# evoldoers/machineboss

Measured on NVIDIA B200. Metric: forward_viterbi_gcups, higher is better.
Workload: dtype f64

## Files before the change

machineboss_b200/csrc/mb_api.cu:

```cuda
#include <algorithm>
#include <cmath>
#include <cstdio>
#include <cstring>
#include <mutex>

#include "mb_internal.h"

namespace mb {

static thread_local std::string g_error;
static thread_local int g_device = 0;
static thread_local int g_forceEngine = -1;
static thread_local Options g_options;

static const char* const kOptionNames[] = {
  "verbose",
  "jit_narrow", "jit_no_linear", "jit_c", "jit_cv", "jit_minblocks", "jit_minblocks_v", "jit_minblocks_linv", "jit_minblocks_lin", "jit_minblocks_cnt", "jit_threads",
  "jit_tb_budget_mb", "jit_f_budget_mb",
  "jit_chunks",
  "jit_no_norm",
  "jit_unroll",
  "jit_fit_c",
  "jit_split",
  "lane_r", "lane_warps", "no_lane", "lane_old", "lane_bs", "lane_la", "lane_wn", "lane_host_only", "lane_warps_per_cta", "wide_g", "wide_w", "no_big", "big_warps", "big_debug", "big_no_fold", "big_early_store", "big_smem_kb",
  "no_col", "col_no_traceback", "col_bp_budget_mb", "col_c", "col_sil_regs", "col_threads", "col_minblocks", "col_r", "col_bnd_budget_mb",
};

Options thread_options() { return g_options; }
void set_thread_options (const Options& o) { g_options = o; }
int thread_engine() { return g_forceEngine; }

bool option_known (const char* name) {
  for (const char* n: kOptionNames) if (!strcmp (n, name)) return true;
  return false;
}

void set_error (const std::string& msg) { g_error = msg; }

bool cuda_ok (cudaError_t e, const char* what) {
  if (e == cudaSuccess) return true;
  set_error (std::string ("CUDA error: ") + cudaGetErrorString (e) + " in " + what);
  return false;
}

int timing_begin (mb_batch* b) {
  b->lastMs = 0;
  b->lastLaunches = 0;
  MB_CUDA (cudaEventRecord (b->evStart, b->stream));
  return 0;
}

int timing_end (mb_batch* b, int64_t launches) {
  MB_CUDA (cudaEventRecord (b->evStop, b->stream));
// ... 797 lines not shown
```

machineboss_b200/csrc/mb_jit.cu:

```cuda
#include <cuda.h>
#include <dlfcn.h>
#include <nvrtc.h>
#include <unistd.h>

#include <algorithm>
#include <cmath>
#include <cstdio>
#include <cstring>
#include <map>
#include <mutex>
#include <sstream>

#include "mb_internal.h"
#include "mb_jit_skeleton.h"

namespace mb {

struct Driver {
  CUresult (*ModuleLoadData) (CUmodule*, const void*) = nullptr;
  CUresult (*ModuleUnload) (CUmodule) = nullptr;
  CUresult (*ModuleGetFunction) (CUfunction*, CUmodule, const char*) = nullptr;
  CUresult (*ModuleGetGlobal) (CUdeviceptr*, size_t*, CUmodule, const char*) = nullptr;
  CUresult (*LaunchKernel) (CUfunction, unsigned, unsigned, unsigned, unsigned, unsigned, unsigned, unsigned, CUstream, void**, void**) = nullptr;
  CUresult (*FuncSetAttribute) (CUfunction, CUfunction_attribute, int) = nullptr;
// ... 62 lines not shown
      || !g_nvrtc.GetProgramLog || !g_nvrtc.DestroyProgram) { set_error ("libnvrtc is missing symbols"); return false; }
  g_nvrtc.ok = true;
  return true;
}

static bool cu_ok (CUresult r, const char* what) {
  if (r == CUDA_SUCCESS) return true;
  const char* s = nullptr;
  if (g_drv.GetErrorString) g_drv.GetErrorString (r, &s);
  set_error (std::string ("CUDA driver error: ") + (s ? s : "?") + " in " + what);
  return false;
}

struct Slot {
  int type, self, other, rank;
  int emitOff = -1;
  int silIdx = -1;
  int idOff = 0;
  int tableSize = 1;
};

struct Program {
  std::vector<Slot> slots;
  std::vector<int> stateSlot0;
  std::vector<int32_t> idTab;
  std::vector<int32_t> emitId;
  std::vector<int32_t> silId;
  int nEmit = 0, nSil = 0;
  int WA = 0, WB = 0;
  std::vector<int> rowOff;
  std::vector<int32_t> rowId;
  std::vector<int> rowSlot;
  std::vector<int> unitSlot;
};

static int table_size (int type, int nIn, int nOut) {
  return type == T_MATCH ? nIn * nOut : type == T_DELETE ? nIn : type == T_INSERT ? nOut : 1;
}

static int label_index (int type, int a, int b, int nOut) {
  return type == T_MATCH ? (a - 1) * nOut + (b - 1) : type == T_DELETE ? a - 1 : type == T_INSERT ? b - 1 : 0;
}

static int trans_type (int a, int b) { return a ? (b ? T_MATCH : T_DELETE) : (b ? T_INSERT : T_SILENT); }

static void build_program (const mb_machine* m, bool forward, Program& p) {
  struct Key { int self, type, other, rank; bool operator< (const Key& k) const { return std::tie (self, type, other, rank) < std::tie (k.self, k.type, k.other, k.rank); } };
  std::map<Key, std::vector<std::pair<int, int>>> groups;
  std::map<std::tuple<int, int, int, int>, int> seen;
  for (int64_t t = 0; t < m->T; ++t) {
    const int type = trans_type (m->in[t], m->out[t]);
    if (type == T_SILENT && m->dst[t] <= m->src[t]) continue;
    const int self = forward ? m->dst[t] : m->src[t], other = forward ? m->src[t] : m->dst[t];
    const int li = label_index (type, m->in[t], m->out[t], m->nOut);
    const int rank = seen[std::make_tuple (self, type, other, li)]++;
    groups[Key { self, type, other, rank }].push_back ({ li, (int) t });
  }
  p.stateSlot0.assign ((size_t) m->S + 1, 0);
  for (auto& g: groups) {
    Slot s;
    s.type = g.first.type; s.self = g.first.self; s.other = g.first.other; s.rank = g.first.rank;
    s.tableSize = table_size (s.type, m->nIn, m->nOut);
    s.idOff = (int) p.idTab.size();
    p.idTab.resize (p.idTab.size() + s.tableSize, -1);
    for (auto& e: g.second) p.idTab[s.idOff + e.first] = e.second;
    if (s.type == T_SILENT) { s.silIdx = p.nSil++; p.silId.push_back (g.second[0].second); }
    else {
      s.emitOff = p.nEmit;
      p.nEmit += s.tableSize;
      p.emitId.resize ((size_t) p.nEmit, -1);
      for (auto& e: g.second) p.emitId[s.emitOff + e.first] = e.second;
    }
    p.stateSlot0[s.self + 1]++;
    p.slots.push_back (s);
  }
  for (int s = 0; s < m->S; ++s) p.stateSlot0[s + 1] += p.stateSlot0[s];
  p.rowOff.assign (p.slots.size(), -1);
  for (size_t k = 0; k < p.slots.size(); ++k) {
    const Slot& sl = p.slots[k];
    if (sl.type == T_MATCH) { p.rowOff[k] = p.WA; p.WA += m->nOut; }
    else if (sl.type == T_DELETE) { p.rowOff[k] = p.WA; p.WA += 1; }
    else if (sl.type == T_INSERT) { p.rowOff[k] = p.WB; p.WB += 1; }
  }
  p.rowId.assign ((size_t) std::max (m->nIn * p.WA + m->nOut * p.WB, 1), -1);
  p.rowSlot.assign (p.rowId.size(), -1);
  for (size_t k = 0; k < p.slots.size(); ++k) {
    const Slot& sl = p.slots[k];
    auto put = [&] (int entry, int label) { p.rowId[entry] = p.idTab[sl.idOff + label]; p.rowSlot[entry] = (int) k; };
    if (sl.type == T_MATCH) { for (int a = 0; a < m->nIn; ++a) for (int b = 0; b < m->nOut; ++b) put (a * p.WA + p.rowOff[k] + b, a * m->nOut + b); }
    else if (sl.type == T_DELETE) { for (int a = 0; a < m->nIn; ++a) put (a * p.WA + p.rowOff[k], a); }
    else if (sl.type == T_INSERT) { for (int b = 0; b < m->nOut; ++b) put (m->nIn * p.WA + b * p.WB + p.rowOff[k], b); }
  }
  p.unitSlot.assign ((size_t) m->S, -1);
  for (int d = 0; d < m->S; ++d)
    for (int k = p.stateSlot0[d]; k < p.stateSlot0[d + 1]; ++k)
      if (p.slots[k].type == T_SILENT) { p.unitSlot[d] = k; break; }
}

struct JitEngine {
  Program fwd, bwd;
  int C = 4, tbBytes = 1, threads = 128, minBlocks = 4, minBlocksLin = 5, minBlocksCnt = 4;
  int CV = 4, minBlocksV = 4;
  int minBlocksLinV = 4;
  CUfunction kViterbiN = nullptr, kForwardLinN = nullptr, kBackwardLinN = nullptr, kViterbiScoreN = nullptr;
  int blocksPerSMN[4] = { 1, 1, 1, 1 };
  CUfunction kViterbiScore = nullptr;
  double* dRowVit = nullptr;
  double* dRowFLinN = nullptr;
  double* dRowBLinN = nullptr;
  std::vector<char> silParamLinN;
  bool normOK = false;
  std::string sourceV;
  struct FitModule { int C = 0; CUmodule mod = nullptr; CUfunction k[4] = { nullptr, nullptr, nullptr, nullptr }; int blocksPerSM[4] = { 1, 1, 1, 1 }; };
  std::vector<FitModule> fit;
  std::vector<int> fitFailed;
  std::string sourceS;
  CUmodule modS = nullptr;
  bool splitTried = false;
  CUfunction kSplit[4] = { nullptr, nullptr, nullptr, nullptr };
  int blocksPerSMS[4] = { 1, 1, 1, 1 };
  std::vector<int> stored;
  int storeQ = 1;
  CUmodule modV = nullptr;
  std::vector<int> shift, bits;
// ... 83 lines not shown
  for (auto& sl: p.slots) isSource[sl.other] = 1;
  for (int d = 0; d < m->S; ++d) {
    const int s0 = p.stateSlot0[d], s1 = p.stateSlot0[d + 1];
    const bool sinkOnly = !isSource[d] && d != 0 && s0 != s1;
    if (s0 == s1 || sinkOnly) o << "  double n" << d << " = mb_neg_inf();\n";
    if (sinkOnly) o << "  if (sink) {\n";
    for (int k = s0; k < s1; ++k) {
      const Slot& sl = p.slots[k];
      std::ostringstream t;
      t << source_expr (sl) << " + ";
      if (sl.type == T_SILENT) t << "P.f[" << sl.silIdx << "]"; else t << row_weight (sl, p.rowOff[k]);
      if (k == s0) o << (sinkOnly ? "  n" : "  double n") << d << " = " << t.str() << ";\n";
      else {
        const unsigned field = (unsigned) ((1ull << J.bits[d]) - 1ull), val = (unsigned) (k - s0);
        o << "  mb_vmax<PTR> (n" << d << ", " << t.str() << ", pk[(sh + " << J.shift[d] << ") >> 5], " << field << "u << ((sh + " << J.shift[d] << ") & 31), "
          << val << "u << ((sh + " << J.shift[d] << ") & 31));\n";
      }
    }
    if (sinkOnly) o << "  }\n";
    if (d == 0) o << "  if (origin) n" << d << " = 0.0;\n";
  }
  for (int d = 0; d < m->S; ++d) o << "  N[" << d << "] = n" << d << ";\n";
  o << "}\n\n";
}

static void gen_cell_row_lin (std::ostringstream& o, const mb_machine* m, const Program& p, bool forward) {
  o << "__device__ __forceinline__ void " << (forward ? "mb_cell_fwd_linr" : "mb_cell_bwd_linr")
    << " (const double (&D)[MB_S], const double (&L)[MB_S], const double (&U)[MB_S], double (&N)[MB_S], "
       "const unsigned ea, const unsigned em, const unsigned ebr, const bool origin, const MBSilN& P) {\n";
  const int originState = forward ? 0 : m->S - 1;
  for (int q = 0; q < m->S; ++q) {
    const int d = forward ? q : m->S - 1 - q;
    const int s0 = p.stateSlot0[d], s1 = p.stateSlot0[d + 1], unit = p.unitSlot[d];
    if (s0 == s1) o << "  double n" << d << " = 0.0;\n";
    if (unit >= 0) o << "  double n" << d << " = " << source_expr (p.slots[unit]) << ";\n";
    bool first = unit < 0;
    for (int k = s0; k < s1; ++k) {
      if (k == unit) continue;
      const Slot& sl = p.slots[k];
      std::ostringstream w;
      if (sl.type == T_SILENT) w << "P." << (forward ? "f" : "b") << "[" << sl.silIdx << "]"; else w << row_weight (sl, p.rowOff[k]);
      if (first) o << "  double n" << d << " = " << source_expr (sl) << " * " << w.str() << ";\n";
      else o << "  n" << d << " = fma (" << source_expr (sl) << ", " << w.str() << ", n" << d << ");\n";
      first = false;
    }
    if (d == originState) o << "  if (origin) n" << d << " = P." << (forward ? "originF" : "originB") << ";\n";
  }
  for (int d = 0; d < m->S; ++d) o << "  N[" << d << "] = n" << d << ";\n";
  o << "}\n\n";
}

static int ctx_count (int type, int C, int nOut) { return type == T_MATCH ? C * nOut : type == T_DELETE ? C : type == T_INSERT ? nOut : 0; }

static void gen_cell_counts (std::ostringstream& o, const mb_machine* m, const JitEngine& J) {
  const Program& p = J.bwd;
  o << "__device__ __forceinline__ void mb_cell_cnt (const double (&D)[MB_S], const double (&L)[MB_S], const double (&U)[MB_S], double (&N)[MB_S], const int a, const int b, const bool origin, const double* __restrict__ E, const MBSil& P, const double (&F)[MB_S], float (&cs)[MB_NSIL_B > 0 ? MB_NSIL_B : 1], float* __restrict__ acc, const int c) {\n";
  for (int q = 0; q < m->S; ++q) {
    const int d = m->S - 1 - q;
    const int s0 = p.stateSlot0[d], s1 = p.stateSlot0[d + 1];
    if (s0 == s1) o << "  double n" << d << " = mb_neg_inf();\n";
    for (int k = s0; k < s1; ++k) {
      const Slot& sl = p.slots[k];
      o << "  const double t" << k << " = " << term_expr (sl, m->nOut, false) << ";\n";
      if (k == s0) o << "  double n" << d << " = t" << k << ";\n";
      else o << "  n" << d << " = mb_lse (n" << d << ", t" << k << ");\n";
      o << "  { const float p = mb_post (F[" << d << "] + t" << k << "); ";
      if (sl.type == T_SILENT) o << "cs[" << sl.silIdx << "] += p; }\n";
      else {
        o << "acc[(" << J.ctxBase[k] << " + ";
        if (sl.type == T_MATCH) o << "c * " << m->nOut << " + b";
        else if (sl.type == T_DELETE) o << "c";
        else o << "b";
        o << ") * 32] += p; }\n";
      }
    }
    if (d == m->S - 1) o << "  if (origin) n" << d << " = 0.0;\n";
// ... 209 lines not shown
      fclose (f);
      if (!ok || rename (tmp.c_str(), cached.c_str())) remove (tmp.c_str());
    }
  }
  if (const char* d = getenv ("MB_JIT_DUMP")) { FILE* f = fopen ((std::string (d) + dumpSuffix + ".cubin").c_str(), "wb"); if (f) { fwrite (cubin.data(), 1, n, f); fclose (f); } }
  return 0;
}

static int compile (mb_machine* m, JitEngine& J) {
  std::vector<char> cubin, cubinV;
  if (nvrtc_compile (J.source, "", cubin, nullptr) || !load_driver()) return 1;
  if (!J.sourceV.empty() && nvrtc_compile (J.sourceV, ".viterbi.cu", cubinV, nullptr)) return 1;
  MB_CUDA (cudaFree (0));
  if (!cu_ok (g_drv.ModuleLoadData (&J.mod, cubin.data()), "cuModuleLoadData")) return 1;
  if (!J.sourceV.empty() && !cu_ok (g_drv.ModuleLoadData (&J.modV, cubinV.data()), "cuModuleLoadData")) return 1;
  if (!cu_ok (g_drv.ModuleGetFunction (&J.kForward, J.mod, "mb_k_forward"), "cuModuleGetFunction")
      || !cu_ok (g_drv.ModuleGetFunction (&J.kBackward, J.mod, "mb_k_backward"), "cuModuleGetFunction")
      || !cu_ok (g_drv.ModuleGetFunction (&J.kViterbi, J.modV ? J.modV : J.mod, "mb_k_viterbi"), "cuModuleGetFunction")
      || !cu_ok (g_drv.ModuleGetFunction (&J.kViterbiScore, J.modV ? J.modV : J.mod, "mb_k_viterbi_score"), "cuModuleGetFunction")
      || !cu_ok (g_drv.ModuleGetFunction (&J.kFStore, J.mod, "mb_k_fstore"), "cuModuleGetFunction")
      || !cu_ok (g_drv.ModuleGetFunction (&J.kBCounts, J.mod, "mb_k_bcounts"), "cuModuleGetFunction")
      || !cu_ok (g_drv.ModuleGetFunction (&J.kForwardLin, J.modV ? J.modV : J.mod, "mb_k_forward_lin"), "cuModuleGetFunction")
      || !cu_ok (g_drv.ModuleGetFunction (&J.kBackwardLin, J.modV ? J.modV : J.mod, "mb_k_backward_lin"), "cuModuleGetFunction")
      || !cu_ok (g_drv.ModuleGetFunction (&J.kFStoreLin, J.mod, "mb_k_fstore_lin"), "cuModuleGetFunction")
      || !cu_ok (g_drv.ModuleGetFunction (&J.kBCountsLin, J.mod, "mb_k_bcounts_lin"), "cuModuleGetFunction")) return 1;
  if (J.modV && (!cu_ok (g_drv.ModuleGetFunction (&J.kViterbiN, J.mod, "mb_k_viterbi"), "cuModuleGetFunction")
                 || !cu_ok (g_drv.ModuleGetFunction (&J.kViterbiScoreN, J.mod, "mb_k_viterbi_score"), "cuModuleGetFunction")
                 || !cu_ok (g_drv.ModuleGetFunction (&J.kForwardLinN, J.mod, "mb_k_forward_lin"), "cuModuleGetFunction")
                 || !cu_ok (g_drv.ModuleGetFunction (&J.kBackwardLinN, J.mod, "mb_k_backward_lin"), "cuModuleGetFunction"))) return 1;
  int dev = 0;
  MB_CUDA (cudaGetDevice (&dev));
  MB_CUDA (cudaDeviceGetAttribute (&J.numSMs, cudaDevAttrMultiProcessorCount, dev));
  CUfunction fn[10] = { J.kForward, J.kBackward, J.kViterbi, J.kFStore, J.kBCounts, J.kForwardLin, J.kBackwardLin, J.kFStoreLin, J.kBCountsLin, J.kViterbiScore };
  const int ne[10] = { J.fwd.nEmit, J.bwd.nEmit, J.fwd.nEmit, J.fwd.nEmit, J.bwd.nEmit, J.fwd.nEmit, J.bwd.nEmit, J.fwd.nEmit, J.bwd.nEmit, J.fwd.nEmit };
  for (int q = 0; q < 10; ++q) {
    const bool needAcc = q == 4 || q == 8;
    J.smemBytes[q] = (size_t) (((ne[q] + 1) & ~1) + (J.threads / 32) * (16 + 32 * (m->S + 1))) * 8
      + (needAcc ? (size_t) (J.threads / 32) * 32 * std::max (J.nCtx, 1) * (q == 8 ? 8 : 4) : 0)
      + (q == 8 ? (size_t) (J.threads / 32) * 2 * (32 * J.C * J.storeQ * 4) * 4 : 0);
    if (!cu_ok (g_drv.FuncSetAttribute (fn[q], CU_FUNC_ATTRIBUTE_MAX_DYNAMIC_SHARED_SIZE_BYTES, (int) J.smemBytes[q]), "cuFuncSetAttribute")) return 1;
    int nb = 0;
    if (!cu_ok (g_drv.OccupancyMaxActiveBlocksPerMultiprocessor (&nb, fn[q], J.threads, J.smemBytes[q]), "occupancy")) return 1;
    J.blocksPerSM[q] = std::max (1, nb);
  }
  if (J.modV) {
    CUfunction fnN[4] = { J.kViterbiN, J.kForwardLinN, J.kBackwardLinN, J.kViterbiScoreN };
    const int qOf[4] = { 2, 5, 6, 9 };
    for (int q = 0; q < 4; ++q) {
      if (!cu_ok (g_drv.FuncSetAttribute (fnN[q], CU_FUNC_ATTRIBUTE_MAX_DYNAMIC_SHARED_SIZE_BYTES, (int) J.smemBytes[qOf[q]]), "cuFuncSetAttribute")) return 1;
      int nb = 0;
      if (!cu_ok (g_drv.OccupancyMaxActiveBlocksPerMultiprocessor (&nb, fnN[q], J.threads, J.smemBytes[qOf[q]]), "occupancy")) return 1;
      J.blocksPerSMN[q] = std::max (1, nb);
    }
  }
  return 0;
}

static int ensure_split_module (mb_machine* m, JitEngine& J) {
  if (J.modS) return 0;
  if (J.splitTried) { set_error ("jit engine: the split-mode module could not be built"); return 1; }
  J.splitTried = true;
  std::vector<char> cubin;
  if (nvrtc_compile (J.sourceS, ".split.cu", cubin, nullptr)) return 1;
  if (!cu_ok (g_drv.ModuleLoadData (&J.modS, cubin.data()), "cuModuleLoadData")) return 1;
  const char* names[4] = { "mb_k_viterbi", "mb_k_forward_lin", "mb_k_backward_lin", "mb_k_viterbi_score" };
  const int qOf[4] = { 2, 5, 6, 9 };
  for (int q = 0; q < 4; ++q) {
// ... 100 lines not shown
struct RowTables { std::vector<double> rowLog, rowLinN, silN; double originInv = 1, resLog = 0; bool ok = true; };

static void row_tables (const mb_machine* m, const Program& p, bool forward, RowTables& r) {
  const int S = m->S;
  const double kLn2 = 0.6931471805599453;
  std::vector<double> ls ((size_t) S, 0.);
  r.ok = true;
  for (int q = 0; q < S; ++q) {
    const int d = forward ? q : S - 1 - q;
    const int u = p.unitSlot[d];
    if (u < 0) continue;
    const double w = m->lw[p.silId[p.slots[u].silIdx]];
    if (!std::isfinite (w)) { r.ok = false; continue; }
    ls[d] = w + ls[p.slots[u].other];
    if (std::fabs (ls[d]) > 100. * kLn2) r.ok = false;
  }
  auto scaled = [&] (int slot, double w) {
    if (!(w > -INFINITY)) return 0.;
    const double lw = w + ls[p.slots[slot].other] - ls[p.slots[slot].self];
    if (!std::isfinite (lw) || std::fabs (lw) > 48. * kLn2) r.ok = false;
    return std::exp (lw);
  };
  r.rowLog.assign (p.rowId.size(), -INFINITY);
  r.rowLinN.assign (p.rowId.size(), 0.);
  for (size_t e = 0; e < p.rowId.size(); ++e) {
    if (p.rowId[e] < 0) continue;
    const double w = m->lw[p.rowId[e]];
    r.rowLog[e] = w + 0.0;
    r.rowLinN[e] = scaled (p.rowSlot[e], w);
  }
  r.silN.assign ((size_t) std::max (p.nSil, 1), 1.);
  for (size_t k = 0; k < p.slots.size(); ++k)
    if (p.slots[k].type == T_SILENT && (int) k != p.unitSlot[p.slots[k].self]) r.silN[p.slots[k].silIdx] = scaled ((int) k, m->lw[p.silId[p.slots[k].silIdx]]);
  const int originState = forward ? 0 : S - 1, resState = forward ? S - 1 : 0;
  r.originInv = std::exp (-ls[originState]);
  r.resLog = ls[resState];
}

static void fill_weights (const mb_machine* m, JitEngine& J, std::vector<double>& ef, std::vector<double>& eb) {
  const double ninf = -INFINITY;
  ef.assign ((size_t) std::max (J.fwd.nEmit, 1), ninf);
  eb.assign ((size_t) std::max (J.bwd.nEmit, 1), ninf);
  for (int q = 0; q < J.fwd.nEmit; ++q) if (J.fwd.emitId[q] >= 0) ef[q] = m->lw[J.fwd.emitId[q]];
  for (int q = 0; q < J.bwd.nEmit; ++q) if (J.bwd.emitId[q] >= 0) eb[q] = m->lw[J.bwd.emitId[q]];
  const int nf = std::max (J.fwd.nSil, 1), nb = std::max (J.bwd.nSil, 1);
  J.silParam.assign ((size_t) (nf + nb) * 8, 0);
  double* sp = (double*) J.silParam.data();
  for (int q = 0; q < J.fwd.nSil; ++q) sp[q] = m->lw[J.fwd.silId[q]] + 0.0;
  for (int q = 0; q < J.bwd.nSil; ++q) sp[nf + q] = m->lw[J.bwd.silId[q]] + 0.0;
  J.silParamLin.assign (J.silParam.size(), 0);
  double* sl = (double*) J.silParamLin.data();
  for (int q = 0; q < nf + nb; ++q) sl[q] = std::exp (sp[q]);
  J.linearOK = true;
  for (double w: m->lw) if (std::isfinite (w) && std::fabs (w) > 24.0 * 0.6931471805599453) J.linearOK = false;
  for (double w: m->lw) if (std::isnan (w) || w == INFINITY) J.linearOK = false;
  if (m->opt.get ("jit_no_linear", 0)) J.linearOK = false;
}

static int upload_row_tables (const mb_machine* m, JitEngine& J) {
  RowTables f, b;
  row_tables (m, J.fwd, true, f);
  row_tables (m, J.bwd, false, b);
  J.normOK = f.ok && b.ok && J.linearOK && !m->opt.get ("jit_no_norm", 0);
  const int nf = std::max (J.fwd.nSil, 1), nb = std::max (J.bwd.nSil, 1);
  J.silParamLinN.assign ((size_t) (nf + nb + 4) * 8, 0);
  double* sn = (double*) J.silParamLinN.data();
// ... 73 lines not shown
    const int n = ctx_count (J.bwd.slots[k].type, J.C, m->nOut);
    if (n) { J.ctxBase[k] = J.nCtx; J.nCtx += n; }
  }

  J.source = module_source (m, J, J.C, 0, J.minBlocks, J.minBlocksLin);
  J.sourceV = J.CV != J.C ? module_source (m, J, J.CV, 1, J.minBlocksV, J.minBlocksLinV) : std::string();
  J.sourceS = "#define MB_SPLIT 1\n" + (J.sourceV.empty() ? J.source : J.sourceV);
}

static std::string module_source (const mb_machine* m, JitEngine& J, int passC, int pass, int passMinBlocks, int passMinBlocksLin) {
  std::ostringstream o;
  o << "// generated by machineboss_b200 (mb_jit.cu) for a machine with " << m->S << " states, " << m->T << " transitions\n";
  if (pass) o << "#define MB_SCORE_MODULE 1\n#define MB_LANE_FRAMES 1\n";
  o << "#define MB_ROWTAB 1\n";
  o << "#define MB_STEADY_UNROLL " << std::max (1, std::min (4, m->opt.get ("jit_unroll", pass ? 2 : 1))) << "\n";
  o << "typedef unsigned char uint8_t;\ntypedef int int32_t;\ntypedef long long int64_t;\ntypedef unsigned long long uint64_t;\n";
  o << "#define MB_S " << m->S << "\n#define MB_C " << passC << "\n#define MB_NIN " << m->nIn << "\n#define MB_NOUT " << m->nOut << "\n";
  o << "#define MB_NEMIT_F " << J.fwd.nEmit << "\n#define MB_NEMIT_B " << J.bwd.nEmit << "\n#define MB_TBBYTES " << J.tbBytes << "\n#define MB_THREADS " << J.threads << "\n";
  unsigned long long liveF = 0, liveB = 0;
  for (auto& sl: J.fwd.slots) if (sl.type != T_SILENT) liveF |= 1ull << sl.other;
  for (auto& sl: J.bwd.slots) if (sl.type != T_SILENT) liveB |= 1ull << sl.other;
  o << "#define MB_LIVE_F " << liveF << "ull\n#define MB_LIVE_B " << liveB << "ull\n";
  { const int cb = passC * J.tbBytes; if (cb != 1 && cb != 2 && cb != 4 && cb != 8 && cb != 16) o << "#define MB_TBPAD " << 16 / J.tbBytes << "\n"; }
  o << "#define MB_MINBLOCKS " << passMinBlocks << "\n#ifdef MB_SPLIT\n#define MB_MINBLOCKS_LIN " << std::min (2, passMinBlocksLin) << "      // (the split-mode sums spill below 170 registers)\n#else\n#define MB_MINBLOCKS_LIN "
    << passMinBlocksLin << "\n#endif\n#define MB_MINBLOCKS_CNT " << J.minBlocksCnt << "\n";
  o << "#define MB_NSIL_B " << J.bwd.nSil << "\n#define MB_NCTX " << std::max (J.nCtx, 1) << "\n";
  o << "typedef " << (J.tbBytes <= 4 ? "unsigned" : "unsigned long long") << " mb_tbword;\n";
  o << "struct MBSil { double f[" << std::max (J.fwd.nSil, 1) << "]; double b[" << std::max (J.bwd.nSil, 1) << "]; };\n";
  o << "__device__ __forceinline__ double mb_neg_inf();\n__device__ __forceinline__ double mb_lse (double, double);\n";
  o << "__device__ __forceinline__ float mb_post (double);\n__device__ __forceinline__ float mb_warp_sum (float);\n__device__ __forceinline__ double mb_warp_sum_d (double);\n\n";
  {
    o << "// MB_ROWCELLS_BEGIN (the host harness of tests/test_jit_rowcells_host.py compiles from here to MB_ROWCELLS_END)\n";
    o << "#define MB_WA_F " << J.fwd.WA << "\n#define MB_WB_F " << J.fwd.WB << "\n#define MB_WA_B " << J.bwd.WA << "\n#define MB_WB_B " << J.bwd.WB << "\n";
    o << "struct MBSilN { double f[" << std::max (J.fwd.nSil, 1) << "]; double b[" << std::max (J.bwd.nSil, 1) << "]; double originF, originB, resLogF, resLogB; };\n";
    o << "#ifndef MB_LDS\n"
         "template<int OFF> __device__ __forceinline__ double mb_lds (const unsigned addr) { double v; asm (\"ld.shared.f64 %0, [%1+%2];\" : \"=d\"(v) : \"r\"(addr), \"n\"(OFF)); return v; }\n"
         "#define MB_LDS(addr, off) mb_lds<off> (addr)\n#endif\n";
    o << "#define MB_PKW " << (passC * J.tbBytes + 3) / 4 << "      // 32-bit words of packed back-pointers per lane and step\n";
    o << "#ifndef MB_HOST_HARNESS\n"
         "// n = max (n, t) with the reference's tie-break (a later candidate wins only if strictly greater); with PTR the\n"
         "// winner's field value replaces the field in `word`: (word & ~field) | val, or a plain OR for a one-bit field\n"
         "template<bool PTR> __device__ __forceinline__ void mb_vmax (double& n, const double t, unsigned& word, const unsigned field, const unsigned val) {\n"
         "  if (!PTR) { if (n < t) n = t; return; }\n"
         "  if (field == val) asm (\"{ .reg .pred p; setp.lt.f64 p, %0, %2; selp.f64 %0, %2, %0, p; @p or.b32 %1, %1, %3; }\" : \"+d\"(n), \"+r\"(word) : \"d\"(t), \"r\"(val));\n"
         "  else asm (\"{ .reg .pred p; setp.lt.f64 p, %0, %2; selp.f64 %0, %2, %0, p; @p lop3.b32 %1, %1, %3, %4, 0xEA; }\" : \"+d\"(n), \"+r\"(word) : \"d\"(t), \"r\"(~field), \"r\"(val));\n"
         "}\n#endif\n\n";
    gen_cell_row_vit (o, m, J.fwd, J);
    gen_cell_row_lin (o, m, J.fwd, true);
    gen_cell_row_lin (o, m, J.bwd, false);
    o << "// MB_ROWCELLS_END\n";
  }
  gen_cell (o, m, J.fwd, true, false, J);
  gen_cell (o, m, J.bwd, false, false, J);
  gen_cell (o, m, J.fwd, true, true, J);
  gen_cell_counts (o, m, J);
  gen_cell_lin (o, m, J.fwd, true);
  gen_cell_lin (o, m, J.bwd, false);
  gen_cell_counts_lin (o, m, J);
  gen_fstore_lin (o, m, J);
  o << kJitSkeleton;
  return o.str();
}

int jit_host_tables (const mb_machine* m, int which, std::vector<double>& out) {
  std::string why;
  if (!jit_supported (m, &why)) { set_error ("machine not eligible for the JIT engine: " + why); return 1; }
  JitEngine J;
  generate (m, J);
  std::vector<double> ef, eb;
  fill_weights (m, J, ef, eb);
// ... 613 lines not shown
```

machineboss_b200/csrc/mb_jit_skeleton.h:

```cpp
#ifndef MB_JIT_SKELETON_H
#define MB_JIT_SKELETON_H

static const char* const kJitSkeleton = R"MBSRC(
#define MB_W (32 * MB_C)
#define MB_FULL 0xffffffffu

struct MBArgs {
  const uint8_t* x; const int64_t* xOff;
  const uint8_t* y; const int64_t* yOff;
  const int64_t* order; int64_t nWork; unsigned long long* counter;
  double* bnd; int64_t bndStride;
  double* result;
  const double* emit;
  uint8_t* tb; const int64_t* tbOff;
  double* F; const int64_t* fOff;        // full Forward matrices [outPos][inPos][state] (modes 2, 3)
  const double* ll;                      // Forward log-likelihood per pair (mode 3)
  double* counts;                        // [nTrans] posterior counts (mode 3)
  const int32_t* idTabB;                 // transition id per backward-program table entry (mode 3)
  int32_t* flag;                         // per pair: 1 = the scaled linear sweep saw a dangerous dynamic range
  unsigned* F32; const int64_t* f32Off;  // linear E-step: high words of the Forward values, [outPos][inPos][state]
  int32_t* ef; const int64_t* efOff;     // linear E-step: frame exponent per (strip, block of MB_RESCALE steps)
  // SPLIT mode (few or long pairs: fewer pairs than resident warps).  A work item is ONE STRIP of a pair,
  // items[w] = pair << 16 | strip, the strips of a pair consecutive in w; the warps that claim them run as a
  // pipeline down the strips: strip s writes its last column to the item's own boundary buffer and publishes in
// ... 54 lines not shown
  for (int d = 16; d > 0; d >>= 1) v += __shfl_xor_sync (MB_FULL, v, d);
  return v;
}

__device__ __forceinline__ void mb_cp_async16 (void* smem, const void* gmem) {
  asm volatile ("cp.async.cg.shared.global [%0], [%1], 16;" :: "r"((unsigned) __cvta_generic_to_shared (smem)), "l"(gmem));
}
__device__ __forceinline__ void mb_cp_async_commit() { asm volatile ("cp.async.commit_group;"); }
__device__ __forceinline__ void mb_cp_async_wait_all() { asm volatile ("cp.async.wait_group 0;" ::: "memory"); }

__device__ __forceinline__ void mb_prefetch_l2 (const void* p) { asm volatile ("prefetch.global.L2 [%0];" :: "l"(p)); }

__device__ __forceinline__ double mb_warp_sum_d (double v) {
#pragma unroll
  for (int d = 16; d > 0; d >>= 1) v += __shfl_xor_sync (MB_FULL, v, d);
  return v;
}

// lane 0 replaces v by the double at a shared-memory address (the staged boundary row); the other lanes keep theirs:
// one predicated load instead of an unconditional load and two selects
__device__ __forceinline__ void mb_lds_lane0 (double& v, const int lane, const unsigned addr) {
  asm volatile ("{ .reg .pred p; setp.eq.s32 p, %1, 0; @p ld.shared.f64 %0, [%2]; }" : "+d"(v) : "r"(lane), "r"(addr));
}

// log of the scale the result state carries in the normalised linear kernels (0 elsewhere)
template<int DIR> __device__ __forceinline__ double mb_res_log (const MBSil&) { return 0.0; }
#ifdef MB_ROWTAB
template<int DIR> __device__ __forceinline__ double mb_res_log (const MBSilN& P) { return DIR ? P.resLogB : P.resLogF; }
#endif

template<bool B> struct MBBool { static constexpr bool value = B; };

template<int DIR> struct MBDir { };
template<> struct MBDir<0> { static const int NE = MB_NEMIT_F; static const int RES = MB_S - 1; };
template<> struct MBDir<1> { static const int NE = MB_NEMIT_B; static const int RES = 0; };

// states whose values are read by later cells (sources of non-silent transition groups); the
// others are temporaries of the cell function and need no shuffle, boundary slot or rescaling
template<int DIR> __device__ __forceinline__ constexpr bool mb_live (int s) { return ((DIR ? MB_LIVE_B : MB_LIVE_F) >> s) & 1ull; }

#define MB_FBLOCK (32 * MB_C * MB_SQ * 4)       // 32-bit words per warp-step block of stored Forward values
#define MB_ROW (MB_S + 1)      // doubles per strip-boundary row: the states + the frame exponent (linear sweeps)

// MODE 0: log-sum-exp score (Forward for DIR 0, Backward for DIR 1); MODE 1: Viterbi + back-pointers;
// MODE 4: Viterbi score only (boss -V without -A: no pointer is formed, packed or stored);
// MODE 2: Forward that also stores every cell (the E-step's ForwardMatrix, counts.cpp:58);
// MODE 3: Backward fused with the posterior-count accumulation of BackwardMatrix::getCounts
//         (backward.cpp:62-87): each transition group's term w + B(dest) is formed once and used
//         both for the Backward log-sum-exp and for exp(F(src) - ll + term).
template<int MODE, int DIR>
__device__ __forceinline__ void mb_run (const MBSil& P, const MBArgs& A) {
  extern __shared__ double mb_smem[];
  double* E = mb_smem;
  const int NE = MBDir<DIR>::NE;
  const int lane = threadIdx.x & 31, warp = threadIdx.x >> 5;
  for (int q = threadIdx.x; q < NE; q += blockDim.x) E[q] = A.emit[q];
  __syncthreads();
#ifdef MB_ROWTAB
  const unsigned eBase = (unsigned) __cvta_generic_to_shared (E);      // the emission weights in row layout (see the generated prelude)
#endif
  // shared memory: emission table | per warp: 128-byte ring of output-row tokens, published a block
  // ahead so that each lane can fetch its next step's token during the current step | per warp: 32 staged boundary rows | per warp: thread-private count
  // accumulators of the emitting transition groups, acc[ctx * 32 + lane] (count kernels only)
  const int nWarps = blockDim.x >> 5;
  uint8_t* ring = (uint8_t*) (mb_smem + ((NE + 1) & ~1)) + warp * 128;
  double* sIn = mb_smem + ((NE + 1) & ~1) + nWarps * 16 + warp * (32 * MB_ROW);
  float* acc = (float*) (mb_smem + ((NE + 1) & ~1) + nWarps * (16 + 32 * MB_ROW)) + warp * (32 * MB_NCTX) + lane;
  const int64_t wslot = (int64_t) blockIdx.x * nWarps + warp;
  double* bndA = A.bnd + wslot * A.bndStride;
  double* bndB = bndA + (A.bndStride >> 1);
  const double NI = mb_neg_inf();
  const unsigned sInAddr = (unsigned) __cvta_generic_to_shared (sIn);

  for (;;) {
    unsigned long long w = 0;
    if (lane == 0) w = atomicAdd (A.counter, 1ULL);
    w = __shfl_sync (MB_FULL, w, 0);
    if ((int64_t) w >= A.nWork) break;
    const bool split = MB_SPLIT && A.items != 0;
    const int64_t item = split ? A.items[w] : 0;
    const int64_t k = split ? (item >> 16) : A.order[w];
    const int64_t x0 = A.xOff[k], y0 = A.yOff[k];
    const int Li = (int) (A.xOff[k + 1] - x0), Lo = (int) (A.yOff[k + 1] - y0);
    const uint8_t* x = A.x + x0;
    const uint8_t* y = A.y + y0;
    const int nStrips = (Li + MB_W) / MB_W;
    // Back-pointers in SWEEP ORDER: one block per (strip, step) holding the 32 lanes' groups of MB_TBLANE bytes (the lane's
// ... 229 lines not shown
// Same strip / skew mapping as mb_run, but cell values are probabilities in FP64, not log-
// probabilities: a transition group is ONE FMA (value * weight) instead of an add plus a
// log-sum-exp, and the sum it computes is the exact log-sum-exp of the log-domain recurrence.
// All live values of the warp share one power-of-two frame 2^ecur.  Every MB_RESCALE steps the warp
// takes the maximum of its live values (one integer max per value on the high word, one REDUX),
// renormalises everything to [1, 2) with an exact power-of-two multiply and adds the shift to ecur;
// in the same step it stages the next MB_RESCALE rows of the previous strip's boundary, each
// carrying its own frame, already converted to the new frame.  log-likelihood = ln(value) + ecur ln 2.
//
// FP64 spans 2^-1022 .. 2^1023.  At every rescale the warp also takes the minimum non-zero value;
// if the spread max/min exceeds 2^700 (a state that is astronomically unlikely next to its
// neighbours but could still matter later), or a boundary row arrives more than 2^900 away from the
// current frame, the pair is flagged and the host re-runs it with the log-domain kernel (mb_run), as
// it does for every pair whose result is -inf.  The host only selects this kernel when every finite
// log-weight lies in [-24 ln 2, 24 ln 2], which bounds the drift between two rescales by 2^-400.
#define MB_RESCALE 16

// MODE 0: score only.  MODE 2 (DIR 0): also store the Forward values for the E-step -- the HIGH WORD
// of each double (sign, 11-bit exponent, 20-bit mantissa, rounded: relative error 2^-21, full FP64
// range), 4 bytes instead of 8, and only for the states an emitting transition enters (the rest of a
// cell follows from those through its silent transitions, mb_fexpand_lin), plus the frame exponent of
// every rescale block.
// MODE 3 (DIR 1): Backward fused with the posterior counts: for each transition group the product
// term = B(dest) * w feeds the Backward sum and, times F(src) * 2^(eF + eB) / Z, the group's count.
template<int MODE, int DIR, class SIL>
__device__ __forceinline__ void mb_run_lin (const SIL& P, const MBArgs& A) {
#ifdef MB_LANE_FRAMES
  constexpr bool LF = MODE == 0;
#else
  constexpr bool LF = false;
#endif
  extern __shared__ double mb_smem[];
  double* E = mb_smem;
  const int NE = MBDir<DIR>::NE;
  const int lane = threadIdx.x & 31, warp = threadIdx.x >> 5;
  for (int q = threadIdx.x; q < NE; q += blockDim.x) E[q] = A.emit[q];
  __syncthreads();
#ifdef MB_ROWTAB
  // score module: the normalised linear weights in row layout (see the generated prelude)
  constexpr bool ROW = MODE == 0;
  const unsigned eBase = (unsigned) __cvta_generic_to_shared (E);
  constexpr unsigned WA8 = (DIR ? MB_WA_B : MB_WA_F) * 8, WB8 = (DIR ? MB_WB_B : MB_WB_F) * 8;
#else
  constexpr bool ROW = false;
#endif
  // shared memory layout as in mb_run; the count accumulators are FP64 here: accd[ctx * 32 + lane]
  const int nWarps = blockDim.x >> 5;
  uint8_t* ring = (uint8_t*) (mb_smem + ((NE + 1) & ~1)) + warp * 128;
  double* sIn = mb_smem + ((NE + 1) & ~1) + nWarps * 16 + warp * (32 * MB_ROW);
  double* accd = mb_smem + ((NE + 1) & ~1) + nWarps * (16 + 32 * MB_ROW) + warp * (32 * MB_NCTX) + lane;
  // MODE 3: two warp-step blocks of stored Forward words, filled by cp.async one step ahead
  unsigned* fstage = (unsigned*) (mb_smem + ((NE + 1) & ~1) + nWarps * (16 + 32 * MB_ROW + 32 * MB_NCTX)) + warp * (2 * MB_FBLOCK);
  const int64_t wslot = (int64_t) blockIdx.x * nWarps + warp;
  double* bndA = A.bnd + wslot * A.bndStride;
  double* bndB = bndA + (A.bndStride >> 1);
  const unsigned sInAddr = (unsigned) __cvta_generic_to_shared (sIn);

  for (;;) {
    unsigned long long w = 0;
    if (lane == 0) w = atomicAdd (A.counter, 1ULL);
    w = __shfl_sync (MB_FULL, w, 0);
    if ((int64_t) w >= A.nWork) break;
    const bool split = MB_SPLIT && A.items != 0;
    const int64_t item = split ? A.items[w] : 0;
    const int64_t k = split ? (item >> 16) : A.order[w];
    const int64_t x0 = A.xOff[k], y0 = A.yOff[k];
    const int Li = (int) (A.xOff[k + 1] - x0), Lo = (int) (A.yOff[k + 1] - y0);
// ... 341 lines not shown
```

Baseline: 6989.

## Inline single-entry emitting states into silent successors via precomputed weight products

States that have a single emitting incoming transition and that no later cell reads get folded into the silent transitions that leave them. The product of the emission weight and the silent weight is precomputed on the host and stored in extra row-table columns, so the state drops out of the generated cell code. This aims to cut per-cell multiplies and register pressure. In exchange the shared-memory emission table grows (capped at 3072 entries), products that overflow the safe range mark the engine as not ok, and volatile shared loads are used to stop the compiler hoisting these weights into registers.

```diff
diff --git a/machineboss_b200/csrc/mb_api.cu b/machineboss_b200/csrc/mb_api.cu
--- a/machineboss_b200/csrc/mb_api.cu
+++ b/machineboss_b200/csrc/mb_api.cu
@@ -19,6 +19,8 @@
   "jit_tb_budget_mb", "jit_f_budget_mb",
   "jit_chunks",
   "jit_no_norm",
+  "jit_inline_regs",
+  "jit_no_inline",
   "jit_unroll",
   "jit_fit_c",
   "jit_split",
diff --git a/machineboss_b200/csrc/mb_jit.cu b/machineboss_b200/csrc/mb_jit.cu
--- a/machineboss_b200/csrc/mb_jit.cu
+++ b/machineboss_b200/csrc/mb_jit.cu
@@ -118,6 +118,9 @@
   std::vector<int32_t> rowId;
   std::vector<int> rowSlot;
   std::vector<int> unitSlot;
+  std::vector<char> inl;
+  std::vector<int> prodOff;
+  std::vector<int> rowProd;
 };
 
 static int table_size (int type, int nIn, int nOut) {
@@ -129,6 +132,41 @@
 }
 
 static int trans_type (int a, int b) { return a ? (b ? T_MATCH : T_DELETE) : (b ? T_INSERT : T_SILENT); }
+
+static void inline_states (const mb_machine* m, bool forward, Program& p) {
+  const int S = m->S;
+  p.inl.assign ((size_t) S, 0);
+  p.prodOff.assign (p.slots.size(), -1);
+  if (m->opt.get ("jit_no_inline", 0)) return;
+  std::vector<char> live ((size_t) S, 0);
+  for (auto& sl: p.slots) if (sl.type != T_SILENT) live[sl.other] = 1;
+  const int originState = forward ? 0 : S - 1, resState = forward ? S - 1 : 0;
+  const int WA0 = p.WA, WB0 = p.WB;
+  bool any = false;
+  for (int d = 0; d < S; ++d) {
+    const int s0 = p.stateSlot0[d];
+    if (live[d] || d == originState || d == resState || p.stateSlot0[d + 1] - s0 != 1 || p.slots[s0].type == T_SILENT) continue;
+    const int type = p.slots[s0].type;
+    int& W = type == T_INSERT ? p.WB : p.WA;
+    const int width = type == T_MATCH ? m->nOut : 1;
+    int n = 0;
+    for (auto& sl: p.slots) n += sl.type == T_SILENT && sl.other == d;
+    if (!n) continue;
+    if (width == 1 && n > 1) W = (W + 1) & ~1;
+    for (size_t k = 0; k < p.slots.size(); ++k)
+      if (p.slots[k].type == T_SILENT && p.slots[k].other == d) { p.prodOff[k] = W; W += width; }
+    p.inl[d] = 1;
+    any = true;
+  }
+  if (!any) return;
+  p.WA = (p.WA + 1) & ~1;
+  p.WB = (p.WB + 1) & ~1;
+  if (m->nIn * p.WA + m->nOut * p.WB > 3072) {
+    p.WA = WA0; p.WB = WB0;
+    p.inl.assign ((size_t) S, 0);
+    p.prodOff.assign (p.slots.size(), -1);
+  }
+}
 
 static void build_program (const mb_machine* m, bool forward, Program& p) {
   struct Key { int self, type, other, rank; bool operator< (const Key& k) const { return std::tie (self, type, other, rank) < std::tie (k.self, k.type, k.other, k.rank); } };
@@ -168,14 +206,23 @@
     else if (sl.type == T_DELETE) { p.rowOff[k] = p.WA; p.WA += 1; }
     else if (sl.type == T_INSERT) { p.rowOff[k] = p.WB; p.WB += 1; }
   }
+  inline_states (m, forward, p);
   p.rowId.assign ((size_t) std::max (m->nIn * p.WA + m->nOut * p.WB, 1), -1);
   p.rowSlot.assign (p.rowId.size(), -1);
+  p.rowProd.assign (p.rowId.size(), -1);
   for (size_t k = 0; k < p.slots.size(); ++k) {
     const Slot& sl = p.slots[k];
     auto put = [&] (int entry, int label) { p.rowId[entry] = p.idTab[sl.idOff + label]; p.rowSlot[entry] = (int) k; };
     if (sl.type == T_MATCH) { for (int a = 0; a < m->nIn; ++a) for (int b = 0; b < m->nOut; ++b) put (a * p.WA + p.rowOff[k] + b, a * m->nOut + b); }
     else if (sl.type == T_DELETE) { for (int a = 0; a < m->nIn; ++a) put (a * p.WA + p.rowOff[k], a); }
     else if (sl.type == T_INSERT) { for (int b = 0; b < m->nOut; ++b) put (m->nIn * p.WA + b * p.WB + p.rowOff[k], b); }
+    if (p.prodOff[k] < 0) continue;
+    const int e = p.stateSlot0[sl.other];
+    auto prod = [&] (int row, int col) { p.rowProd[row + p.prodOff[k] + col] = row + p.rowOff[e] + col; p.rowSlot[row + p.prodOff[k] + col] = (int) k; };
+    const int type = p.slots[e].type;
+    if (type == T_MATCH) { for (int a = 0; a < m->nIn; ++a) for (int b = 0; b < m->nOut; ++b) prod (a * p.WA, b); }
+    else if (type == T_DELETE) { for (int a = 0; a < m->nIn; ++a) prod (a * p.WA, 0); }
+    else { for (int b = 0; b < m->nOut; ++b) prod (m->nIn * p.WA + b * p.WB, 0); }
   }
   p.unitSlot.assign ((size_t) m->S, -1);
   for (int d = 0; d < m->S; ++d)
@@ -325,16 +372,43 @@
   for (int q = 0; q < m->S; ++q) {
     const int d = forward ? q : m->S - 1 - q;
     const int s0 = p.stateSlot0[d], s1 = p.stateSlot0[d + 1], unit = p.unitSlot[d];
+    if (p.inl[d]) {
+      const Slot& e = p.slots[s0];
+      const bool regs = m->opt.get ("jit_inline_regs", 0);
+      const char* reg = e.type == T_MATCH ? "em" : e.type == T_DELETE ? "ea" : "ebr";
+      std::vector<int> ks;
+      for (size_t k = 0; k < p.slots.size(); ++k) if (p.prodOff[k] >= 0 && p.slots[k].other == d) ks.push_back ((int) k);
+      for (size_t j = 0; j < ks.size(); ++j) {
+        const int off = p.prodOff[ks[j]];
+        if (e.type != T_MATCH && j + 1 < ks.size() && (off & 1) == 0 && p.prodOff[ks[j + 1]] == off + 1) {
+          o << "  double w" << ks[j] << ", w" << ks[j + 1] << ";\n  MB_LDS2" << (regs ? "R" : "") << " (" << reg << ", " << off * 8 << ", w" << ks[j] << ", w" << ks[j + 1] << ");\n";
+          ++j;
+        } else o << "  const double w" << ks[j] << " = MB_LDS" << (regs ? "" : "V") << " (" << reg << ", " << off * 8 << ");\n";
+      }
+      o << "  const double n" << d << " = 0.0;\n";
+      continue;
+    }
     if (s0 == s1) o << "  double n" << d << " = 0.0;\n";
-    if (unit >= 0) o << "  double n" << d << " = " << source_expr (p.slots[unit]) << ";\n";
+    auto term = [&] (int k, std::string& src, std::string& w) {
+      const Slot& sl = p.slots[k];
+      if (p.prodOff[k] >= 0) { src = source_expr (p.slots[p.stateSlot0[sl.other]]); w = "w" + std::to_string (k); return; }
+      src = source_expr (sl);
+      std::ostringstream ws;
+      if (sl.type == T_SILENT) ws << "P." << (forward ? "f" : "b") << "[" << sl.silIdx << "]"; else ws << row_weight (sl, p.rowOff[k]);
+      w = ws.str();
+    };
+    std::string src, w;
+    if (unit >= 0) {
+      term (unit, src, w);
+      if (p.prodOff[unit] >= 0) o << "  double n" << d << " = " << src << " * " << w << ";\n";
+      else o << "  double n" << d << " = " << src << ";\n";
+    }
     bool first = unit < 0;
     for (int k = s0; k < s1; ++k) {
       if (k == unit) continue;
-      const Slot& sl = p.slots[k];
-      std::ostringstream w;
-      if (sl.type == T_SILENT) w << "P." << (forward ? "f" : "b") << "[" << sl.silIdx << "]"; else w << row_weight (sl, p.rowOff[k]);
-      if (first) o << "  double n" << d << " = " << source_expr (sl) << " * " << w.str() << ";\n";
-      else o << "  n" << d << " = fma (" << source_expr (sl) << ", " << w.str() << ", n" << d << ");\n";
+      term (k, src, w);
+      if (first) o << "  double n" << d << " = " << src << " * " << w << ";\n";
+      else o << "  n" << d << " = fma (" << src << ", " << w << ", n" << d << ");\n";
       first = false;
     }
     if (d == originState) o << "  if (origin) n" << d << " = P." << (forward ? "originF" : "originB") << ";\n";
@@ -610,7 +684,8 @@
   MB_CUDA (cudaGetDevice (&dev));
   MB_CUDA (cudaDeviceGetAttribute (&J.numSMs, cudaDevAttrMultiProcessorCount, dev));
   CUfunction fn[10] = { J.kForward, J.kBackward, J.kViterbi, J.kFStore, J.kBCounts, J.kForwardLin, J.kBackwardLin, J.kFStoreLin, J.kBCountsLin, J.kViterbiScore };
-  const int ne[10] = { J.fwd.nEmit, J.bwd.nEmit, J.fwd.nEmit, J.fwd.nEmit, J.bwd.nEmit, J.fwd.nEmit, J.bwd.nEmit, J.fwd.nEmit, J.bwd.nEmit, J.fwd.nEmit };
+  const int nrF = (int) J.fwd.rowId.size(), nrB = (int) J.bwd.rowId.size();
+  const int ne[10] = { J.fwd.nEmit, J.bwd.nEmit, nrF, J.fwd.nEmit, J.bwd.nEmit, nrF, nrB, J.fwd.nEmit, J.bwd.nEmit, nrF };
   for (int q = 0; q < 10; ++q) {
     const bool needAcc = q == 4 || q == 8;
     J.smemBytes[q] = (size_t) (((ne[q] + 1) & ~1) + (J.threads / 32) * (16 + 32 * (m->S + 1))) * 8
@@ -777,6 +852,12 @@
   r.silN.assign ((size_t) std::max (p.nSil, 1), 1.);
   for (size_t k = 0; k < p.slots.size(); ++k)
     if (p.slots[k].type == T_SILENT && (int) k != p.unitSlot[p.slots[k].self]) r.silN[p.slots[k].silIdx] = scaled ((int) k, m->lw[p.silId[p.slots[k].silIdx]]);
+  for (size_t e = 0; e < p.rowProd.size(); ++e) {
+    if (p.rowProd[e] < 0) continue;
+    const double v = r.rowLinN[p.rowProd[e]] * r.silN[p.slots[p.rowSlot[e]].silIdx];
+    if (v != 0. && std::fabs (std::log2 (v)) > 100.) r.ok = false;
+    r.rowLinN[e] = v;
+  }
   const int originState = forward ? 0 : S - 1, resState = forward ? S - 1 : 0;
   r.originInv = std::exp (-ls[originState]);
   r.resLog = ls[resState];
@@ -916,10 +997,20 @@
   {
     o << "// MB_ROWCELLS_BEGIN (the host harness of tests/test_jit_rowcells_host.py compiles from here to MB_ROWCELLS_END)\n";
     o << "#define MB_WA_F " << J.fwd.WA << "\n#define MB_WB_F " << J.fwd.WB << "\n#define MB_WA_B " << J.bwd.WA << "\n#define MB_WB_B " << J.bwd.WB << "\n";
+    o << "#define MB_NROW_F " << J.fwd.rowId.size() << "\n#define MB_NROW_B " << J.bwd.rowId.size() << "\n";
     o << "struct MBSilN { double f[" << std::max (J.fwd.nSil, 1) << "]; double b[" << std::max (J.bwd.nSil, 1) << "]; double originF, originB, resLogF, resLogB; };\n";
     o << "#ifndef MB_LDS\n"
          "template<int OFF> __device__ __forceinline__ double mb_lds (const unsigned addr) { double v; asm (\"ld.shared.f64 %0, [%1+%2];\" : \"=d\"(v) : \"r\"(addr), \"n\"(OFF)); return v; }\n"
-         "#define MB_LDS(addr, off) mb_lds<off> (addr)\n#endif\n";
+         "#define MB_LDS(addr, off) mb_lds<off> (addr)\n"
+         "// the products of inlined states (inline_states), read in every cell: volatile, so that the compiler does not keep a\n"
+         "// strip's worth of them in registers (with 8 columns per lane that pushes the sums past their register budget)\n"
+         "template<int OFF> __device__ __forceinline__ double mb_ldsv (const unsigned addr) { double v; asm volatile (\"ld.shared.f64 %0, [%1+%2];\" : \"=d\"(v) : \"r\"(addr), \"n\"(OFF)); return v; }\n"
+         "#define MB_LDSV(addr, off) mb_ldsv<off> (addr)\n"
+         "template<int OFF> __device__ __forceinline__ void mb_lds2 (const unsigned addr, double& v0, double& v1) { asm volatile (\"ld.shared.v2.f64 {%0, %1}, [%2+%3];\" : \"=d\"(v0), \"=d\"(v1) : \"r\"(addr), \"n\"(OFF)); }\n"
+         "#define MB_LDS2(addr, off, v0, v1) mb_lds2<off> (addr, v0, v1)\n"
+         "template<int OFF> __device__ __forceinline__ void mb_lds2r (const unsigned addr, double& v0, double& v1) { asm (\"ld.shared.v2.f64 {%0, %1}, [%2+%3];\" : \"=d\"(v0), \"=d\"(v1) : \"r\"(addr), \"n\"(OFF)); }\n"
+         "#define MB_LDS2R(addr, off, v0, v1) mb_lds2r<off> (addr, v0, v1)\n#endif\n"
+         "#ifndef MB_LDS2\n#define MB_LDSV MB_LDS\n#define MB_LDS2(addr, off, v0, v1) (v0 = MB_LDS (addr, off), v1 = MB_LDS (addr, (off) + 8))\n#define MB_LDS2R MB_LDS2\n#endif\n";
     o << "#define MB_PKW " << (passC * J.tbBytes + 3) / 4 << "      // 32-bit words of packed back-pointers per lane and step\n";
     o << "#ifndef MB_HOST_HARNESS\n"
          "// n = max (n, t) with the reference's tie-break (a later candidate wins only if strictly greater); with PTR the\n"
diff --git a/machineboss_b200/csrc/mb_jit_skeleton.h b/machineboss_b200/csrc/mb_jit_skeleton.h
--- a/machineboss_b200/csrc/mb_jit_skeleton.h
+++ b/machineboss_b200/csrc/mb_jit_skeleton.h
@@ -110,8 +110,9 @@
 template<bool B> struct MBBool { static constexpr bool value = B; };
 
 template<int DIR> struct MBDir { };
-template<> struct MBDir<0> { static const int NE = MB_NEMIT_F; static const int RES = MB_S - 1; };
-template<> struct MBDir<1> { static const int NE = MB_NEMIT_B; static const int RES = 0; };
+// NE: entries of the indexed emission table; NR: of the row-layout table (which also holds the products of inlined states)
+template<> struct MBDir<0> { static const int NE = MB_NEMIT_F; static const int NR = MB_NROW_F; static const int RES = MB_S - 1; };
+template<> struct MBDir<1> { static const int NE = MB_NEMIT_B; static const int NR = MB_NROW_B; static const int RES = 0; };
 
 // states whose values are read by later cells (sources of non-silent transition groups); the
 // others are temporaries of the cell function and need no shuffle, boundary slot or rescaling
@@ -130,7 +131,11 @@
 __device__ __forceinline__ void mb_run (const MBSil& P, const MBArgs& A) {
   extern __shared__ double mb_smem[];
   double* E = mb_smem;
+#ifdef MB_ROWTAB
+  const int NE = (MODE == 1 || MODE == 4) ? MBDir<DIR>::NR : MBDir<DIR>::NE;
+#else
   const int NE = MBDir<DIR>::NE;
+#endif
   const int lane = threadIdx.x & 31, warp = threadIdx.x >> 5;
   for (int q = threadIdx.x; q < NE; q += blockDim.x) E[q] = A.emit[q];
   __syncthreads();
@@ -426,7 +431,11 @@
 #endif
   extern __shared__ double mb_smem[];
   double* E = mb_smem;
+#ifdef MB_ROWTAB
+  const int NE = MODE == 0 ? MBDir<DIR>::NR : MBDir<DIR>::NE;
+#else
   const int NE = MBDir<DIR>::NE;
+#endif
   const int lane = threadIdx.x & 31, warp = threadIdx.x >> 5;
   for (int q = threadIdx.x; q < NE; q += blockDim.x) E[q] = A.emit[q];
   __syncthreads();
```

New measurement: 5983 (median of 6 runs). 14.4% lower.
